# this-Demir/3D-Ray-Tracer-Vulkan

Hardware: AMD Instinct MI355X
Metric: Mrays/s at 1920×1080×4-bounce, 50k-tri scene; 1/2/4/8 GPU + %HBM roofline (higher is better)
Workload: dtype f32

## Files before the change

### 3d-ray-tracer-vulkan_amd/csrc/rt_internal.h

```cpp
#pragma once
#include <cstdint>
#include <cstddef>
#include <hip/hip_runtime.h>

#include "../../include/rtamd.h"

namespace rtamd {

constexpr int kShadeStride = 2;

struct DevScene {
    int      n_nodes = 0;
    int      end     = 0;
    int      n_tris  = 0;
    int      root_leaf = 0;
    float    root_box[6] = {0, 0, 0, 0, 0, 0};
    float4*  nodes   = nullptr;
    float4*  leafs   = nullptr;
    float4*  pairs   = nullptr;
    float4*  walk    = nullptr;
    int*     slot_node = nullptr;
    int*     node_slot = nullptr;
    int      end2    = 0;
    int      padded  = 0;
// ... 5 lines not shown
    int      root_enter = 0;
    int      root_first_leaf = 0;
    int      oct_mask = 7;
    float4*  walk_ref = nullptr;
    int      end2_ref = 0;
    int      ref_padded = 0;
    float4*  norms   = nullptr;
    float4*  mats    = nullptr;
    const float4* spheres = nullptr;
    int      n_spheres = 0;
};

struct Counters {
    unsigned long long segments;
    unsigned long long node_visits;
    unsigned long long tri_tests;
    unsigned long long mat_reads;
};

struct CamF {
    float ox, oy, oz;
    float lx, ly, lz;
    float hx, hy, hz;
    float vx, vy, vz;
};

constexpr int kExtSkyToggle = 1;
constexpr int kExtEmissive = 2;
constexpr int kExtAccumulate = 4;
constexpr int kExtSpheres = 8;
constexpr int kExtNewSample = 16;

constexpr int kMaxBatch = 16;

struct TraceArgs {
    DevScene scene;
    CamF     cams[kMaxBatch];
    int      n_frames;
    int      tiles_y;
    int      width, height;
    int      max_bounces;
    int      x0, y0, tw, th;
    int      band_h, band_stride, band_off;
    const int* band_list;
    uchar4*  out_rgba;
    float*   out_rad;
    Counters* counters;
    int      wave_tile;
    unsigned long long* diag;
    int      coop_lanes;
    int      solo_lanes;
    int      ext;
    int      sky_enabled;
    int      frame_count;
    float*   accum;
    int      walk;
    int      block_waves;
    const int* tile_order;
    int      tiles_x;
    int      split_n;
    int      heavy_tiles;
    int      heavy_fused;
    const int* heavy_px;
    int      n_heavy_px;
    const unsigned long long* tile_mask;
    unsigned* diag_lane;
    hipStream_t aux_stream;
    hipEvent_t ev_fork, ev_join;
    int      coop_walk;
    int      coop_win = 64;
    int      list_stride;
    const int* row_off = nullptr;
    int      split_bounce = 0;
    float4*  q_slots = nullptr;
    unsigned* q_count = nullptr;
    unsigned* q_prefix = nullptr;
    int      q_waves = 0;
    int      q_grid = 0;
    void*    q_temp = nullptr;
    size_t   q_temp_bytes = 0;
    const float4* ray_in = nullptr;
    float4*  hit_out = nullptr;
    int      any_hit = 0;
};

struct HostScene {
    int n_nodes = 0, end = 0, n_tris = 0, max_depth = 0, root_leaf = 0;
    float root_box[6] = {0, 0, 0, 0, 0, 0};
    float4* nodes = nullptr;
    float4* leafs = nullptr;
    float4* pairs = nullptr;
    float4* norms = nullptr;
    float4* mats  = nullptr;
};
int build_host_scene(const void* vertices, size_t vertex_bytes,
                     const void* materials, size_t material_bytes,
                     const void* bvh_nodes, size_t bvh_bytes,
                     HostScene* out, const char** err);
void free_host_scene(HostScene* s);

constexpr unsigned kLearnHeavyMark = 0x3FFFFFFFu;

struct LearnParams {
    int      n;
    int      rec_off;
    int      learn_cost;
    int      order_split;
    int      heavy_pixel_factor;
    int      concurrent;
    int      resident;
    int      cap;
    int      xcd = 0;
    int      tiles_x = 0, tiles_y = 0, frames = 0;
// ... 73 lines not shown
```

### 3d-ray-tracer-vulkan_amd/csrc/rt_runtime.hip

```cpp
#include "rt_internal.h"
#include <rocprim/device/device_scan.hpp>

#include "accel_build.h"

#include <cmath>
#include <cstdarg>
#include <cstdio>
#include <cstdlib>
#include <algorithm>
#include <cstring>
#include <new>
#include <string>
#include <vector>

namespace rtamd {

static thread_local char g_err[1024] = "";

void set_error(const char* fmt, ...) {
    va_list ap;
    va_start(ap, fmt);
    vsnprintf(g_err, sizeof g_err, fmt, ap);
    va_end(ap);
}

#define RT_HIP_CHECK(expr)                                                        \
    do {                                                                          \
        hipError_t e_ = (expr);                                                   \
        if (e_ != hipSuccess) {                                                   \
            set_error("%s failed: %s (%s:%d)", #expr, hipGetErrorString(e_),      \
                      __FILE__, __LINE__);                                        \
            return RT_ERR_HIP;                                                    \
        }                                                                         \
    } while (0)
// ... 208 lines not shown
                   bool pending = false;
                   void* d_base = nullptr;
                   int* d_nhpix = nullptr;
                   rt_learn_params given = {};
                   bool xcd_applied = false;
                   uint64_t seq = 0; };
    void*        d_learn_scratch = nullptr;
    size_t       learn_scratch_cap = 0;
    int*         h_nhpix = nullptr;
    hipEvent_t   learn_ev = nullptr;
    bool         learn_busy = false;
    bool         learn_oom = false;
    bool         learning_device = false;
    int          learning_rec_off = 0;
    uint64_t     learn_seq = 0;
    hipStream_t  aux[4] = {nullptr, nullptr, nullptr, nullptr};
    hipEvent_t   aux_fork[4] = {nullptr, nullptr, nullptr, nullptr}, aux_join[4] = {nullptr, nullptr, nullptr, nullptr};
    unsigned     aux_next = 0;
    std::vector<Order> orders;
    std::vector<uint8_t> learning_key;
    struct LastCam { std::vector<uint8_t> geo; std::vector<uint8_t> cam; };
    std::vector<LastCam> last_cam;
    size_t       learning_n = 0;
    int          learning_tx = 0, learning_ty = 0, learning_frames = 0;
    int          last_heavy = 0;
    int          last_heavy_px = 0;
    int          last_solo = 0;
    struct Graph { std::vector<uint64_t> key; hipGraphExec_t exec; int kernels; };
    uint64_t     plain_kernels = 0;
    struct BandList { std::vector<int> bands; int* d; };
    std::vector<BandList> band_lists;
    std::vector<Graph> graphs;
    unsigned     graph_next = 0;
    struct Slots { hipStream_t s; char* base; int waves; size_t temp_bytes; };
    std::vector<Slots> slots;
    char*        d_query = nullptr;
    size_t       query_cap = 0;
    int          ref_root_leaf = 0;
    char*        d_denoise = nullptr;
    size_t       denoise_cap = 0;
    char*        d_temporal = nullptr;
    size_t       temporal_cap = 0;
    bool         temporal_valid = false;
    int          temporal_last = 0, temporal_w = 0, temporal_h = 0;
    rt_camera_ubo temporal_cam = {};
    bool         moments_valid = false;
};

static constexpr size_t kMaxOrders = 16;
static constexpr int    kResidentPerCu = 24;
static constexpr int    kMaxHeavy = 256;
static constexpr size_t kWin32Bytes = 32ull << 20;
static constexpr size_t kSplitSlotBytes = 256ull << 20;
static constexpr unsigned kMaxWalkSlots = (1u << 27) - 4;
static constexpr size_t kDiagWords = 8;

static void free_order(PerDevice::Order& o) {
    if (o.d_base) {
        (void)hipFree(o.d_base);
        return;
    }
    (void)hipFree(o.d_order);
    if (o.d_hpix) (void)hipFree(o.d_hpix);
    if (o.d_mask) (void)hipFree(o.d_mask);
}

static void poll_learning(PerDevice& p) {
    if (!p.learn_busy || hipEventQuery(p.learn_ev) != hipSuccess) return;
    for (auto& o : p.orders)
        if (o.pending) {
            o.n_hpix = std::max(0, *p.h_nhpix);
            o.pending = false;
        }
    p.learn_busy = false;
}

static void free_orders(PerDevice& p) {
    for (auto& o : p.orders) free_order(o);
    p.orders.clear();
}

static void free_graphs(PerDevice& p) {
    for (auto& g : p.graphs) (void)hipGraphExecDestroy(g.exec);
    p.graphs.clear();
}
static constexpr size_t kMaxGraphs = 64;
// ... 5 lines not shown
    int  wave_tile = -1;
    int  diag = 0;
    int  coop_lanes = -1;
    int  solo_lanes = -1;
    int  ext = 0;
    int  new_sample = 0;
    int  walk = 2;
    int  coop_walk = 0;
    int  coop_window = 0;
    int  block_waves = 1;
    int  heavy_first = 1;
    int  heavy_factor = 130;
    int  heavy_pixels = 1;
    int  heavy_pixel_factor = 50;
    int  reuse_order = 1;
    int  heavy_cap = 75;
    int  async_slots = 4;
    int  copy_streams = 1;
    int  in_async = 0;
    int  concurrent_launches = 1;
    int  learn_cost = 1;
    int  learn_alone = 0;
    int  accel_octants = 7;
    int  xcd_order = 0;
    int  learn_device = 1;
    int  leaf_align = 2;
    int  accel_half = 0;
    int  accel_wide = 0;
    int  denoise_kernel = 0;
    int  denoise_pass = -1;
    int  temporal_tile = 0;
    int  variance_stage = -1;
    int  split_bounce = 0;
    int  accel = 8;
    int  order_split = 0;
    int  order_frames = 0;
    int  graph = 1;
    int  heavy_stream = 2;
    int  heavy_tiles = -1;
    uint64_t scene_gen = 0;
    int  hw_queues = 4;
    bool has_scene = false;
    int  n_nodes = 0, n_tris = 0, max_depth = 0;
    uint64_t issued = 0;
};

static void free_scene(PerDevice& p) {
    if (p.scene.nodes) (void)hipFree(p.scene.nodes);
    if (p.scene.leafs) (void)hipFree(p.scene.leafs);
    if (p.scene.walk) (void)hipFree(p.scene.walk);
    if (p.scene.walk_ref) (void)hipFree(p.scene.walk_ref);
    if (p.scene.slot_node) (void)hipFree(p.scene.slot_node);
    if (p.scene.node_slot) (void)hipFree(p.scene.node_slot);
    if (p.scene.pairs) (void)hipFree(p.scene.pairs);
    if (p.scene.norms) (void)hipFree(p.scene.norms);
    p.scene = DevScene{};
}

static int concurrency(const rt_ctx* ctx) { return std::max(ctx->concurrent_launches, ctx->in_async); }

static int plan_order(const rt_ctx* ctx, PerDevice& p, TraceArgs& a, const rt_camera_ubo* cams,
                      const std::vector<int>* bands) {
    a.tile_order = nullptr;
    a.tiles_x = 0;
    a.split_n = 0;
    a.heavy_tiles = 0;
// ... 359 lines not shown
        const size_t split = ctx->heavy_first ? (size_t)(ctx->heavy_tiles < 0 ? kMaxHeavy : ctx->heavy_tiles) * 63 : 0;
        const size_t words = (waves + split) * 8;
        if (words > p.diag_cap) {
            if (p.d_diag) {
                RT_HIP_CHECK(hipDeviceSynchronize());
                (void)hipFree(p.d_diag);
            }
            p.d_diag = nullptr;
            p.diag_cap = 0;
            RT_HIP_CHECK(hipMalloc(&p.d_diag, words * sizeof(unsigned long long)));
            p.diag_cap = words;
        }
        p.diag_used = words;
        a.diag = p.d_diag;
    }
    return plan_order(ctx, p, a, cam, bands);
}

static std::vector<uint64_t> launch_key(const TraceArgs& a, hipStream_t s) {
    auto P = [](const void* q) { return (uint64_t)(uintptr_t)q; };
    auto F = [](float f) { uint32_t u; std::memcpy(&u, &f, 4); return (uint64_t)u; };
    const DevScene& sc = a.scene;
    std::vector<uint64_t> k = {P(s), P(sc.nodes), P(sc.leafs), P(sc.pairs), P(sc.walk), P(sc.slot_node), P(sc.node_slot), P(sc.norms), P(sc.mats), P(sc.spheres),
            (uint64_t)sc.n_spheres, (uint64_t)sc.n_nodes, (uint64_t)sc.end, (uint64_t)sc.end2, (uint64_t)sc.n_tris,
            (uint64_t)sc.root_leaf, F(sc.root_box[0]), F(sc.root_box[1]), F(sc.root_box[2]), F(sc.root_box[3]),
            F(sc.root_box[4]), F(sc.root_box[5]), (uint64_t)a.n_frames, P(a.band_list), (uint64_t)a.list_stride,
            (uint64_t)a.width, (uint64_t)a.height, (uint64_t)a.max_bounces, (uint64_t)a.x0, (uint64_t)a.y0,
            (uint64_t)a.tw, (uint64_t)a.th, (uint64_t)a.band_h, (uint64_t)a.band_stride, (uint64_t)a.band_off,
            P(a.out_rgba), P(a.out_rad), (uint64_t)a.wave_tile,
            (uint64_t)a.coop_lanes, (uint64_t)a.solo_lanes, (uint64_t)a.ext, (uint64_t)a.sky_enabled,
            (uint64_t)a.frame_count, P(a.accum), (uint64_t)a.walk, (uint64_t)a.block_waves, P(a.tile_order),
            (uint64_t)a.heavy_tiles, (uint64_t)(a.aux_stream != nullptr), (uint64_t)a.heavy_fused, P(a.heavy_px),
            (uint64_t)a.n_heavy_px, P(a.tile_mask), (uint64_t)a.coop_walk, (uint64_t)a.coop_win,
            (uint64_t)a.split_bounce, P(a.q_slots), (uint64_t)a.q_waves, (uint64_t)a.q_grid};
    for (int f = 0; f < a.n_frames; ++f) {
        const CamF& c = a.cams[f];
        for (float v : {c.ox, c.oy, c.oz, c.lx, c.ly, c.lz, c.hx, c.hy, c.hz, c.vx, c.vy, c.vz}) k.push_back(F(v));
    }
    return k;
}

static int attach_slots(const rt_ctx* ctx, PerDevice& p, TraceArgs& a, hipStream_t s) {
    a.q_slots = nullptr;
    a.split_bounce = 0;
    if (!p.scene.n_layouts || ctx->split_bounce <= 0 || ctx->split_bounce >= a.max_bounces || a.ext || a.diag ||
        a.counters)
        return RT_OK;
    const int tw_w = 8 << a.wave_tile, th_w = 8 >> a.wave_tile, bw = std::max(1, a.block_waves);
    const long long waves = (long long)((a.tw + bw * tw_w - 1) / (bw * tw_w)) * bw *
                            ((a.th + th_w - 1) / th_w) * (long long)a.n_frames;
    if (waves > (1 << 24) || (size_t)waves * 64 * 48 > kSplitSlotBytes) return RT_OK;
    PerDevice::Slots* q = nullptr;
    for (auto& x : p.slots)
        if (x.s == s) { q = &x; break; }
    if (!q || q->waves < waves) {
        if (q) {
            RT_HIP_CHECK(hipStreamSynchronize(s));
            (void)hipFree(q->base);
            q->base = nullptr;
            q->waves = 0;
        } else {
            p.slots.push_back(PerDevice::Slots{s, nullptr, 0, 0});
            q = &p.slots.back();
        }
        size_t tb = 0;
        RT_HIP_CHECK(rocprim::exclusive_scan(nullptr, tb, (const unsigned*)nullptr, (unsigned*)nullptr, 0u,
                                             (size_t)waves, rocprim::plus<unsigned>()));
        void* base = nullptr;
        const size_t bytes = (size_t)waves * 64 * 48 + 2 * ((size_t)waves * 4 + 256) + tb + 256;
        RT_HIP_CHECK(hipMalloc(&base, bytes));
        q->base = static_cast<char*>(base);
        q->waves = (int)waves;
        q->temp_bytes = tb;
    }
    a.split_bounce = ctx->split_bounce;
    a.q_slots = reinterpret_cast<float4*>(q->base);
    a.q_count = reinterpret_cast<unsigned*>(q->base + (size_t)q->waves * 64 * 48);
    a.q_prefix = reinterpret_cast<unsigned*>(reinterpret_cast<char*>(a.q_count) + (size_t)q->waves * 4 + 256);
    a.q_temp = reinterpret_cast<char*>(a.q_prefix) + (size_t)q->waves * 4 + 256;
    a.q_temp_bytes = q->temp_bytes;
    a.q_waves = q->waves;
    a.q_grid = std::max(1, p.n_cu * 32);
    return RT_OK;
}

static int launch(const rt_ctx* ctx, PerDevice& p, const TraceArgs& a_in, hipStream_t s) {
    TraceArgs a = a_in;
    if (int rq = attach_slots(ctx, p, a, s)) return rq;
    const bool plain = !a.counters && !a.diag;
    int nk = 1;
    if (!ctx->graph || s == nullptr || a.counters || a.diag || !a.aux_stream) {
        RT_HIP_CHECK(launch_trace(a, s, &nk));
        if (plain) p.plain_kernels += (uint64_t)nk;
        return RT_OK;
    }
    std::vector<uint64_t> key = launch_key(a, s);
    for (auto& g : p.graphs)
        if (g.key == key) {
            RT_HIP_CHECK(hipGraphLaunch(g.exec, s));
            p.plain_kernels += g.kernels;
            return RT_OK;
        }
    hipGraph_t graph = nullptr;
    RT_HIP_CHECK(hipStreamBeginCapture(s, hipStreamCaptureModeThreadLocal));
    const hipError_t le = launch_trace(a, s, &nk);
    const hipError_t ce = hipStreamEndCapture(s, &graph);
    if (le != hipSuccess || ce != hipSuccess) {
        if (graph) (void)hipGraphDestroy(graph);
        set_error("graph capture: %s", hipGetErrorString(le != hipSuccess ? le : ce));
        return RT_ERR_HIP;
    }
    hipGraphExec_t exec = nullptr;
    const hipError_t ie = hipGraphInstantiate(&exec, graph, nullptr, nullptr, 0);
    (void)hipGraphDestroy(graph);
    if (ie != hipSuccess) { set_error("graph instantiate: %s", hipGetErrorString(ie)); return RT_ERR_HIP; }
    if (p.graphs.size() >= kMaxGraphs) {
        const size_t k = p.graph_next++ % kMaxGraphs;
        (void)hipGraphExecDestroy(p.graphs[k].exec);
        p.graphs[k] = PerDevice::Graph{std::move(key), exec, nk};
    } else {
        p.graphs.push_back(PerDevice::Graph{std::move(key), exec, nk});
    }
    RT_HIP_CHECK(hipGraphLaunch(exec, s));
    p.plain_kernels += (uint64_t)nk;
    return RT_OK;
}
// ... 1665 lines not shown
    return {name, field, 0, -1, 3, {a, b, c}};
}
static const Option kOptions[] = {
    in_range("coop_lanes", &rt_ctx::coop_lanes, -1, 64),
    in_range("solo_lanes", &rt_ctx::solo_lanes, -1, 64),
    in_range("extensions", &rt_ctx::ext, 0, 15),
    one_of("new_sample", &rt_ctx::new_sample, 0, 1),
    one_of("walk", &rt_ctx::walk, 0, 2),
    one_of("coop_window", &rt_ctx::coop_window, 0, 32, 64),
    one_of("coop_walk", &rt_ctx::coop_walk, 0, 1),
    one_of("block_waves", &rt_ctx::block_waves, 1, 4),
    one_of("heavy_first", &rt_ctx::heavy_first, 0, 1),
    in_range("heavy_tiles", &rt_ctx::heavy_tiles, -1, 1 << 20),
    in_range("heavy_factor", &rt_ctx::heavy_factor, 10, 100000),
    one_of("heavy_pixels", &rt_ctx::heavy_pixels, 0, 1),
    in_range("heavy_pixel_factor", &rt_ctx::heavy_pixel_factor, 1, 100000),
    one_of("reuse_order", &rt_ctx::reuse_order, 0, 1),
    in_range("heavy_cap", &rt_ctx::heavy_cap, 1, 100),
    in_range("async_slots", &rt_ctx::async_slots, 1, kMaxSlots),
    one_of("copy_streams", &rt_ctx::copy_streams, 1, 2),
    in_range("concurrent_launches", &rt_ctx::concurrent_launches, 1, 64),
    one_of("learn_cost", &rt_ctx::learn_cost, 0, 1),
    one_of("order_frames", &rt_ctx::order_frames, 0, 1),
    in_range("order_split", &rt_ctx::order_split, 0, 100),
    one_of("learn_alone", &rt_ctx::learn_alone, 0, 1),
    in_range("xcd_order", &rt_ctx::xcd_order, 0, 4096),
    in_range("accel_octants", &rt_ctx::accel_octants, 0, 7),
    one_of("learn_device", &rt_ctx::learn_device, 0, 1),
    in_range("leaf_align", &rt_ctx::leaf_align, 0, 2),
    one_of("accel", &rt_ctx::accel, 0, 1, 8),
    one_of("accel_half", &rt_ctx::accel_half, 0, 1),
    one_of("accel_wide", &rt_ctx::accel_wide, 0, 1),
    in_range("split_bounce", &rt_ctx::split_bounce, 0, 64),
    in_range("heavy_stream", &rt_ctx::heavy_stream, 0, 2),
    one_of("graph", &rt_ctx::graph, 0, 1),
    one_of("diag", &rt_ctx::diag, 0, 1),
    in_range("wave_tile", &rt_ctx::wave_tile, -1, 3),
    in_range("denoise_kernel", &rt_ctx::denoise_kernel, 0, 2),
    in_range("denoise_pass", &rt_ctx::denoise_pass, -1, 5),
    in_range("temporal_tile", &rt_ctx::temporal_tile, 0, 2),
    in_range("variance_stage", &rt_ctx::variance_stage, -1, 0),
};

static const Option* find_option(const char* name) {
    for (const Option& o : kOptions)
        if (std::strcmp(name, o.name) == 0) return &o;
    return nullptr;
}

int rt_set_option(rt_ctx* ctx, const char* name, int64_t value) {
    if (!ctx || !name) { set_error("rt_set_option: null argument"); return RT_ERR_INVALID_ARG; }
    static const char* const archived[] = {"shade_min", "blocks_per_cu", "seg_limit", "heavy_budget", "prio_after"};
    for (const char* a : archived)
        if (std::strcmp(name, a) == 0) {
            set_error("rt_set_option: %s belonged to a schedule archived in round 3 (profiles/r03/archive)", name);
            return RT_ERR_INVALID_ARG;
        }
    if (std::strcmp(name, "kernel") == 0 && value == 0) return RT_OK;
    if (const Option* o = find_option(name)) {
        bool ok = value >= o->lo && value <= o->hi;
        for (int k = 0; k < o->n; ++k) ok = ok || value == o->set[k];
        if (ok) {
            ctx->*(o->field) = (int)value;
            return RT_OK;
        }
    }
    set_error("rt_set_option: unknown option or bad value: %s = %lld", name, (long long)value);
    return RT_ERR_INVALID_ARG;
}

int rt_get_option(rt_ctx* ctx, const char* name, int64_t* value) {
    if (!ctx || !name || !value) { set_error("rt_get_option: null argument"); return RT_ERR_INVALID_ARG; }
    if (const Option* o = find_option(name)) {
        *value = ctx->*(o->field);
        return RT_OK;
    }
    const auto is = [name](const char* s) { return std::strcmp(name, s) == 0; };
    PerDevice* p = ctx->dev.empty() ? nullptr : &ctx->dev[0];
    if (is("kernel")) *value = 0;
    else if (is("wave_tile_used")) *value = p ? wave_tile_of(ctx, *p) : 0;
    else if (is("coop_window_used")) *value = p ? coop_window_of(ctx, *p) : 0;
    else if (is("accel_half_used")) *value = p ? p->scene.half : 0;
    else if (is("accel_wide_used")) *value = p ? p->scene.wide : 0;
    else if (is("accel_used")) *value = p ? p->scene.n_layouts : 0;
    else if (is("walk_bytes")) *value = p ? (int64_t)walk_bytes(*p) : 0;
    else if (is("leaf_align_used")) *value = p ? p->scene.padded : 0;
    else if (is("heavy_pixels_used")) *value = p ? p->last_heavy_px : 0;
    else if (is("heavy_tiles_used")) *value = p ? p->last_heavy : 0;
    else if (is("solo_lanes_used")) *value = p ? p->last_solo : 0;
    else if (is("plain_kernels")) *value = p ? (int64_t)p->plain_kernels : 0;
    else if (is("hw_queues")) *value = ctx->hw_queues;
    else if (is("queues_short")) *value = ctx->async_slots + 2 > ctx->hw_queues ? 1 : 0;
    else { set_error("rt_get_option: unknown option %s", name); return RT_ERR_INVALID_ARG; }
    return RT_OK;
}

int rt_diag_copy(rt_ctx* ctx, void* dst, size_t cap_words, size_t* n_words) {
    if (!ctx || !n_words) { set_error("rt_diag_copy: null argument"); return RT_ERR_INVALID_ARG; }
    PerDevice& p = ctx->dev[0];
    *n_words = p.diag_used;
    if (dst && p.d_diag && p.diag_used) {
        RT_HIP_CHECK(hipSetDevice(p.device));
        RT_HIP_CHECK(hipDeviceSynchronize());
        RT_HIP_CHECK(hipMemcpy(dst, p.d_diag, std::min(cap_words, p.diag_used) * 8, hipMemcpyDeviceToHost));
    }
    return RT_OK;
}

int rt_learn_device(rt_ctx* ctx, const void* d_records, const void* d_lanes, int n_tiles, const rt_learn_params* params,
                    void* d_order, void* d_mask, void* d_hpix, void* d_count, void* stream) {
    if (!ctx || !d_records || !d_lanes || !params || !d_order || !d_mask || !d_count) {
        set_error("rt_learn_device: null argument");
        return RT_ERR_INVALID_ARG;
    }
    const rt_learn_params& g = *params;
    if (n_tiles < 1 || n_tiles > (1 << 24) || g.rec_off < 0 || g.rec_off > (1 << 24) || (g.learn_cost & ~1) ||
        g.order_split < 0 || g.order_split > 100 || g.heavy_pixel_factor < 1 || g.concurrent < 1 || g.resident < 1 ||
        g.cap < 0 || g.xcd < 0 || g.tiles_x < 0 || g.tiles_y < 0 || g.frames < 0 || (g.cap > 0 && !d_hpix)) {
        set_error("rt_learn_device: bad tile count or parameters");
        return RT_ERR_INVALID_ARG;
    }
    PerDevice& p = ctx->dev[0];
    RT_HIP_CHECK(hipSetDevice(p.device));
// ... 139 lines not shown
```

### 3d-ray-tracer-vulkan_amd/csrc/rt_trace.hip

```cpp
#include <algorithm>
#include <cstdio>
#include <cstdlib>
#include <cstring>

#include <rocprim/device/device_scan.hpp>

#include "rt_internal.h"

namespace rtamd {

namespace {

constexpr float kTMin = 0.001f;
constexpr float kTMax = 10000.0f;
constexpr int   kMaxRejectTriples = 1 << 16;

struct V3 { float x, y, z; };

__device__ __forceinline__ V3 vadd(V3 a, V3 b) { return {a.x + b.x, a.y + b.y, a.z + b.z}; }
__device__ __forceinline__ V3 vsub(V3 a, V3 b) { return {a.x - b.x, a.y - b.y, a.z - b.z}; }
__device__ __forceinline__ V3 vmul(V3 a, V3 b) { return {a.x * b.x, a.y * b.y, a.z * b.z}; }
__device__ __forceinline__ V3 vscale(V3 a, float s) { return {a.x * s, a.y * s, a.z * s}; }
__device__ __forceinline__ float vdot(V3 a, V3 b) { return (a.x * b.x + a.y * b.y) + a.z * b.z; }
__device__ __forceinline__ V3 vcross(V3 a, V3 b) {
    return {a.y * b.z - a.z * b.y, a.z * b.x - a.x * b.z, a.x * b.y - a.y * b.x};
}
__device__ __forceinline__ V3 vnormalize(V3 a) {
    const float l = sqrtf(vdot(a, a));
    return {a.x / l, a.y / l, a.z / l};
}

__device__ __forceinline__ uint32_t pcg(uint32_t v) {
    const uint32_t s = v * 747796405u + 2891336453u;
    const uint32_t w = ((s >> ((s >> 28u) + 4u)) ^ s) * 277803737u;
    return (w >> 22u) ^ w;
}
__device__ __forceinline__ float rnd(uint32_t& seed) {
    seed = pcg(seed);
// ... 729 lines not shown
            }
        }
        sl = nl;
        if (!(sb < se)) break;
        if (QRY && any_hit && ((__ballot(hit >= 0 && !incons) >> L) & 1ull) != 0ull) break;
    }
    if (me) {
        if (COUNT) {
            c_node += cn;
            c_tri += ct;
        }
        if (DIAG) d_iters += steps;
    }
}

constexpr int kWavesPerEu = 8;
constexpr int kWalkPrio = 2;
template <bool COUNT, bool DIAG = false, int FEAT = 0, int WALK = 2>
__global__ __launch_bounds__(256)
__attribute__((amdgpu_waves_per_eu((FEAT & kFeatFrontier) ? 1 : kWavesPerEu)))
void trace_simple(TraceArgs a) {
    constexpr bool ACC = (FEAT & kFeatAccel) != 0;
    constexpr bool HALF = ACC && (FEAT & kFeatHalf) != 0;
    constexpr bool WIDE = ACC && (FEAT & kFeatWide) != 0;
    constexpr bool PAD = !ACC && ((FEAT & kFeatPad) || (FEAT & (kFeatExt | kFeatFrontier)) || !(FEAT & kFeatCoopTail));
    constexpr bool Q1 = (FEAT & kFeatQ1) != 0, Q2 = (FEAT & kFeatQ2) != 0;
    constexpr bool QRY = (FEAT & kFeatQuery) != 0;
    constexpr bool SOLO = (FEAT & kFeatSolo) != 0;
    static_assert(!SOLO || (ACC && !HALF && !WIDE && WALK == 2 && !(FEAT & (kFeatCoopTail | kFeatExt))),
                  "kFeatSolo goes with the format-0 accel walk alone");
    const int lane = threadIdx.x & 63;
    const int wave = threadIdx.x >> 6;
    extern __shared__ uint4 fr[];
    unsigned q_k = Q2 ? blockIdx.x : 0u;
    const unsigned q_total = Q2 ? a.q_prefix[a.q_waves - 1] + a.q_count[a.q_waves - 1] : 0u;
    if (Q2 && q_k * 64u >= q_total) return;
    const int s = a.wave_tile;
    const int tw_w = 8 << s, th_w = 8 >> s;
    int bx = blockIdx.x, by = blockIdx.y, sub = -1;
    if (QRY) {
        by = bx / a.tiles_x;
        bx -= by * a.tiles_x;
    }
    unsigned long long skip_lanes = 0;
    const int k_wave = (blockIdx.y * gridDim.x + blockIdx.x) * a.block_waves + wave;
    int rec_id = k_wave, tile_id = k_wave, hq = -1;
    if (a.tile_order) {
        const int k = blockIdx.x;
        int t;
        if ((FEAT & kFeatFused) && k < a.n_heavy_px) {
            hq = a.heavy_px[k];
            t = hq >> 6;
            sub = hq & 63;
        } else if (k < 64 * a.split_n) {
            t = a.tile_order[k >> 6];
            sub = k & 63;
        } else {
            t = a.tile_order[k - 63 * a.split_n - ((FEAT & kFeatFused) ? a.n_heavy_px : 0)];
            if ((FEAT & kFeatFused) && a.tile_mask) skip_lanes = a.tile_mask[t];
            if (FEAT & kFeatFused) {
                rec_id = a.n_heavy_px + t;
                tile_id = t;
            } else if (DIAG && a.diag_lane && a.split_n == 0) {
                rec_id = t;
                tile_id = t;
            }
        }
        bx = t % a.tiles_x;
        by = t / a.tiles_x;
    }
    unsigned long long* drec = nullptr;
    if (DIAG) {
        drec = a.diag + kDiagWords * (size_t)rec_id;
        diag_stamp(drec, 0);
    }
    if ((FEAT & kFeatFused) && sub >= 0) {
        const int hf = by / a.tiles_y;
        const int hy = (by - hf * a.tiles_y) * th_w + (sub >> (3 + s));
        heavy_pixel<COUNT>(a, hf, bx * tw_w + (sub & (tw_w - 1)), hy, (a.row_off ? a.row_off[hf] : hf * a.th) + hy, fr);
        if (DIAG) {
            diag_stamp(drec, 1);
            if (lane == 0) {
                drec[4] = 0;
                drec[5] = 0;
                drec[6] = 0;
                drec[7] = 0;
                if (a.diag_lane && hq >= 0) a.diag_lane[hq] = kHeavyLaneMark;
            }
        }
        return;
    }
    const int tl = sub >= 0 ? sub : lane;
    const int col = bx * a.block_waves + wave;
    const int fr_i = by / a.tiles_y;
    by -= fr_i * a.tiles_y;
    int lx = col * tw_w + (tl & (tw_w - 1));
    const int ly = by * th_w + (tl >> (3 + s));
    int lyo = (a.row_off ? a.row_off[fr_i] : fr_i * a.th) + ly;
    const bool pixel = !Q2 && lx < a.tw && ly < a.th && (sub < 0 || lane == 0) && !((skip_lanes >> lane) & 1ull) &&
                       (a.list_stride == 0 || a.band_list[fr_i * a.list_stride + ly / a.band_h] >= 0);
    if (Q1 && lane == 0) a.q_count[k_wave] = 0u;
    const int coop_lanes = sub >= 0 ? 64 : a.coop_lanes;
    const float4* __restrict__ nodes = a.scene.nodes;
    const float4* __restrict__ leafs = a.scene.leafs;
    const float4* __restrict__ pairs = a.scene.pairs;
    const int end = a.scene.end;
    const int wend = WALK == 2 ? a.scene.end2 : end;
    unsigned long long c_seg = 0, c_node = 0, c_tri = 0, c_mat = 0;
    unsigned long long d_iters = 0, d_windows = 0, d_coop_t = 0;
    unsigned long long d_lane_windows = 0;

  do {
    uint32_t seed = 0;
    V3 o = {0.f, 0.f, 0.f}, d = {0.f, 0.f, 1.f};
    V3 att = {1.0f, 1.0f, 1.0f};
    bool alive = pixel;
    int b0 = 0;
    float tmax = kTMax;
    bool refq = false;
    if (Q2) {
        const unsigned i = q_k * 64u + (unsigned)lane;
        alive = i < q_total;
        b0 = a.split_bounce;
        if (alive) {
            int lo = 0, hi = a.q_waves;
            while (hi - lo > 1) {
                const int mid = (lo + hi) >> 1;
                if (a.q_prefix[mid] <= i) lo = mid;
                else hi = mid;
            }
            const float4* r = a.q_slots + 3 * ((size_t)lo * 64 + (i - a.q_prefix[lo]));
            const float4 r0 = r[0], r1 = r[1], r2 = r[2];
            o = {r0.x, r0.y, r0.z};
            d = {r0.w, r1.x, r1.y};
            att = {r1.z, r1.w, r2.x};
            seed = __float_as_uint(r2.y);
            const int pq = __float_as_int(r2.z);
            lyo = pq / a.tw;
            lx = pq - lyo * a.tw;
        }
    }
    if (QRY && a.ray_in) {
        if (pixel) {
            const float4 r0 = a.ray_in[2 * (size_t)lx], r1 = a.ray_in[2 * (size_t)lx + 1];
            o = {r0.x, r0.y, r0.z};
            d = {r1.x, r1.y, r1.z};
            if (r0.w < kTMax) tmax = r0.w;
            if (!finite3(o) || !finite3(d) || (d.x == 0.0f && d.y == 0.0f && d.z == 0.0f)) {
                store_hit(a.hit_out + 2 * (size_t)lx, 0.0f, -2, V3{0.f, 0.f, 0.f}, V3{0.f, 0.f, 0.f});
                alive = false;
            }
            refq = ACC && fabsf(vdot(d, d) - 1.0f) > kRelaxAbs;
        }
    } else if (pixel) {
        const int x = a.x0 + lx, y = frame_row(a, fr_i, ly);
        if ((FEAT & kFeatExt) && (a.ext & (kExtAccumulate | kExtNewSample))) {
            seed = (uint32_t)(y * a.width + x) + (uint32_t)a.frame_count * (uint32_t)(a.width * a.height);
            primary_ray_seeded(a, fr_i, x, y, seed, o, d);
        } else {
            primary_ray(a, fr_i, x, y, seed, o, d);
        }
    }

    for (int b = b0; b < (QRY ? 1 : a.max_bounces); ++b) {
        if (__ballot(alive) == 0) break;
        if (Q1 && b == a.split_bounce) {
            const uint64_t m = __ballot(alive);
            if (alive) {
                float4* r = a.q_slots + 3 * ((size_t)k_wave * 64 + (size_t)lanes_below(m));
                r[0] = make_float4(o.x, o.y, o.z, d.x);
                r[1] = make_float4(d.y, d.z, att.x, att.y);
                r[2] = make_float4(att.z, __uint_as_float(seed), __int_as_float(lyo * a.tw + lx), 0.0f);
            }
            if (lane == 0) a.q_count[k_wave] = (unsigned)__popcll(m);
            alive = false;
            break;
        }
        float closest = QRY ? tmax : kTMax;
        int hit = -1;
        const V3 inv = {1.0f / d.x, 1.0f / d.y, 1.0f / d.z};
        int n = 0;
        int lend = wend;
        bool incons = false;
        int oct = 0;
        if (ACC && a.scene.n_layouts == 8) {
            oct = (int)((__float_as_uint(d.x) >> 31) | ((__float_as_uint(d.y) >> 31) << 1) |
                        ((__float_as_uint(d.z) >> 31) << 2)) & a.scene.oct_mask;
            n = oct * a.scene.layout_slots;
            lend = n + a.scene.layout_slots;
        }
        bool nleaf = a.scene.root_leaf != 0;
        const bool own = alive && !(QRY && refq);
        bool walking = own && end > 0;
        if (ACC && !HALF && !WIDE && a.scene.root_enter) {
            n += 1;
            nleaf = ((a.scene.root_first_leaf >> oct) & 1) != 0;
            if (COUNT && own) c_node += 2;
        }
        uint32_t wcur = a.scene.root_leaf ? kWLeaf : 0u;
        int wsp = 0;
        bool wovf = false;
        if (COUNT && alive) {
            ++c_seg;
            if (end > 0 && own) ++c_node;
        }
        {
            float4 A, B, Q0, Q1;
            const float4* __restrict__ wr = a.scene.walk;
            const __amdgpu_buffer_rsrc_t wrs = __builtin_amdgcn_make_buffer_rsrc(
// ... 227 lines not shown
            if ((FEAT & kFeatExt) ? hit != -1 : hit >= 0) {
                if (COUNT) ++c_mat;
                const V3 hp = vadd(o, vscale(d, closest));
                V3 nrm;
                float4 M;
                if ((FEAT & kFeatExt) && hit < -1) {
                    nrm = sphere_normal(a.scene.spheres[2 * (-2 - hit)], hp, d);
                    M = a.scene.spheres[2 * (-2 - hit) + 1];
                } else {
                    nrm = hit_normal(a.scene.norms, hit, d);
                    M = a.scene.mats[kShadeStride * hit];
                }
                V3 nd;
                if ((FEAT & kFeatExt) && (a.ext & kExtEmissive) && M.w == 3.0f) {
                    fin = vmul(att, V3{M.x, M.y, M.z});
                    alive = false;
                } else if (!scatter(M, d, nrm, seed, nd)) {
                    alive = false;
                } else {
                    att = vmul(att, V3{M.x, M.y, M.z});
                    o = hp;
                    d = nd;
                    if (b == a.max_bounces - 1) alive = false;
                }
            } else {
                if (!((FEAT & kFeatExt) && (a.ext & kExtSkyToggle) && a.sky_enabled == 0))
                    fin = vmul(att, sky_color(d));
                alive = false;
            }
            if (!alive) finish_pixel<FEAT>(a, lx, lyo, fin);
        }
    }
    if (!QRY && alive) finish_pixel<FEAT>(a, lx, lyo, V3{0.0f, 0.0f, 0.0f});
    q_k += gridDim.x;
  } while (Q2 && q_k * 64u < q_total);
    if (COUNT) flush_counters(a.counters, c_seg, c_node, c_tri, c_mat);
    if (DIAG) {
        diag_stamp(drec, 1);
        if (a.diag_lane && !((skip_lanes >> lane) & 1ull))
            a.diag_lane[(size_t)tile_id * 64 + lane] = (unsigned)(d_iters + 2 * d_lane_windows);
        unsigned long long d_sum = d_iters;
#pragma unroll
        for (int off = 32; off > 0; off >>= 1) {
            d_sum += __shfl_xor(d_sum, off);
            const unsigned long long o2 = __shfl_xor(d_iters, off);
            d_iters = o2 > d_iters ? o2 : d_iters;
        }
        if (lane == 0) {
            drec[4] = d_iters;
            drec[5] = d_windows;
            drec[6] = d_coop_t;
            drec[7] = d_sum;
        }
    }
}

}

#define RT_FUSED(G)                                                                                           \
    if (a.diag) hipLaunchKernelGGL((trace_simple<false, true, FF, 2>), G, block, shm, stream, ao);             \
    else if (a.counters) hipLaunchKernelGGL((trace_simple<true, false, FF, 2>), G, block, shm, stream, ao);     \
    else hipLaunchKernelGGL((trace_simple<false, false, FF, 2>), G, block, shm, stream, ao);
#define RT_FUSED_BIG(G)                                                                                       \
    switch (big) {                                                                                            \
        case kFeatWin32: { constexpr int FF = kFeatCoopTail | kFeatFused | kFeatWin32; RT_FUSED(G) } break;   \
        case kFeatPad: { constexpr int FF = kFeatCoopTail | kFeatFused | kFeatPad; RT_FUSED(G) } break;       \
        case kFeatWin32 | kFeatPad: {                                                                         \
            constexpr int FF = kFeatCoopTail | kFeatFused | kFeatWin32 | kFeatPad;                            \
// ... 47 lines not shown
                if (e != hipSuccess) return e;
            }
            TraceArgs ah = ao;
            ah.split_n = H;
            ah.coop_walk = 1;
            const dim3 gh(64 * H);
            const size_t shm = kFCap * sizeof(uint4);
            constexpr int FH = kFeatCoopTail | kFeatFrontier;
            if (a.diag) hipLaunchKernelGGL((trace_simple<false, true, FH, 2>), gh, block, shm, hs, ah);
            else if (a.counters) hipLaunchKernelGGL((trace_simple<true, false, FH, 2>), gh, block, shm, hs, ah);
            else hipLaunchKernelGGL((trace_simple<false, false, FH, 2>), gh, block, shm, hs, ah);
            e = hipGetLastError();
            if (e == hipSuccess && a.aux_stream) e = hipEventRecord(a.ev_join, a.aux_stream);
            if (e != hipSuccess) return e;
            if (kernels) *kernels = 2;
            ao.tile_order = a.tile_order + H;
            if (a.diag) ao.diag = a.diag + (size_t)kDiagWords * gh.x;
            grid = dim3(n_tiles - H);
            join = a.aux_stream != nullptr;
        } else {
            grid = dim3(n_tiles);
        }
    }
    const size_t shm_f = (size_t)bw * kFCap * sizeof(uint4);
    const size_t shm_w = (size_t)bw * kWideStackK * 64 * 6;
#define RT_SHM(F) (((F) & kFeatFrontier) ? shm_f : ((F) & kFeatWide) ? shm_w : 0)
#define RT_SIMPLE(F, W)                                                                                         \
    if (a.diag) hipLaunchKernelGGL((trace_simple<false, true, F, W>), grid, block, RT_SHM(F), stream, ao);           \
    else if (a.counters) hipLaunchKernelGGL((trace_simple<true, false, F, W>), grid, block, RT_SHM(F), stream, ao); \
    else hipLaunchKernelGGL((trace_simple<false, false, F, W>), grid, block, RT_SHM(F), stream, ao);
    if (a.scene.n_layouts > 0) {
        if (a.q_slots && a.split_bounce > 0 && a.split_bounce < a.max_bounces && feat == 0 && !a.scene.half &&
            !a.scene.wide &&
            !a.diag && !a.counters && (int)(grid.x * grid.y) * bw <= a.q_waves) {
            ao.q_waves = (int)(grid.x * grid.y) * bw;
            if (a.solo_lanes > 0)
                hipLaunchKernelGGL((trace_simple<false, false, kFeatAccel | kFeatQ1 | kFeatSolo, 2>), grid, block, 0,
                                   stream, ao);
            else
                hipLaunchKernelGGL((trace_simple<false, false, kFeatAccel | kFeatQ1, 2>), grid, block, 0, stream, ao);
            size_t tb = a.q_temp_bytes;
            const hipError_t se = rocprim::exclusive_scan(a.q_temp, tb, a.q_count, a.q_prefix, 0u,
                                                          (size_t)ao.q_waves, rocprim::plus<unsigned>(), stream);
            if (se != hipSuccess) return se;
            TraceArgs a2 = ao;
            a2.tile_order = nullptr;
            a2.split_n = 0;
            a2.block_waves = 1;
            if (a.solo_lanes > 0)
                hipLaunchKernelGGL((trace_simple<false, false, kFeatAccel | kFeatQ2 | kFeatSolo, 2>), dim3(a.q_grid),
                                   dim3(64), 0, stream, a2);
            else
                hipLaunchKernelGGL((trace_simple<false, false, kFeatAccel | kFeatQ2, 2>), dim3(a.q_grid), dim3(64), 0,
                                   stream, a2);
            if (kernels) *kernels = 2;
            return hipGetLastError();
        }
        if (a.scene.wide) {
            if (feat & kFeatCoopTail) {
                set_error("accel_wide launch with coop_lanes %d", a.coop_lanes);
                return hipErrorInvalidValue;
            }
            if (feat & kFeatExt) RT_SIMPLE(kFeatExt | kFeatAccel | kFeatWide, 2)
            else RT_SIMPLE(kFeatAccel | kFeatWide, 2)
            return hipGetLastError();
        }
        if (a.scene.half) {
            if (feat & kFeatCoopTail) {
                set_error("accel_half launch with coop_lanes %d", a.coop_lanes);
                return hipErrorInvalidValue;
            }
            if (feat & kFeatExt) RT_SIMPLE(kFeatExt | kFeatAccel | kFeatHalf, 2)
            else RT_SIMPLE(kFeatAccel | kFeatHalf, 2)
            return hipGetLastError();
        }
        switch (feat & ~kFeatFrontier) {
            case kFeatCoopTail:
                if (a.coop_win == 32) RT_SIMPLE(kFeatCoopTail | kFeatAccel | kFeatWin32, 2)
                else RT_SIMPLE(kFeatCoopTail | kFeatAccel, 2)
                break;
            case 0:
                if (a.solo_lanes > 0) RT_SIMPLE(kFeatAccel | kFeatSolo, 2)
                else RT_SIMPLE(kFeatAccel, 2)
                break;
            default: RT_SIMPLE(kFeatCoopTail | kFeatExt | kFeatAccel, 2) break;
        }
// ... 65 lines not shown
```

Measured before the change: 32550.

## Replace scan-based ray compaction with atomic bounded queues and auto-enable split

Wavefront ray compaction at the split bounce now appends surviving rays into a fixed set of bounded queues with atomic counters, replacing the per-wave count array, rocPRIM exclusive scan and binary-search lookup. The second pass launches one 64-lane block per queue pack, reads each ray directly, and resets the queue headers with a ticket counter, so no scan kernel or persistent loop is needed. Splitting at bounce 2 is also switched on by default for large frames with at least three bounces. Waves that find their queue full keep tracing in the first pass and bump an overflow counter. The risks are atomic contention, uneven fill across queues, and the new default changing which path runs.

```diff
diff --git a/3d-ray-tracer-vulkan_amd/csrc/rt_internal.h b/3d-ray-tracer-vulkan_amd/csrc/rt_internal.h
--- a/3d-ray-tracer-vulkan_amd/csrc/rt_internal.h
+++ b/3d-ray-tracer-vulkan_amd/csrc/rt_internal.h
@@ -61,6 +61,12 @@
 constexpr int kExtNewSample = 16;
 
 constexpr int kMaxBatch = 16;
+
+constexpr int kQHdrWords = 32;
+constexpr int kQCount = 0;
+constexpr int kQLimit = 1;
+constexpr int kQTicket = 2;
+constexpr int kMaxSplitQueues = 1024;
 
 struct TraceArgs {
     DevScene scene;
@@ -102,12 +108,13 @@
     const int* row_off = nullptr;
     int      split_bounce = 0;
     float4*  q_slots = nullptr;
-    unsigned* q_count = nullptr;
-    unsigned* q_prefix = nullptr;
-    int      q_waves = 0;
-    int      q_grid = 0;
-    void*    q_temp = nullptr;
-    size_t   q_temp_bytes = 0;
+    unsigned* q_hdr = nullptr;
+    unsigned* q_overflow = nullptr;
+    int      q_queues = 0;
+    int      q_cap = 0;
+    unsigned long long q_pixels = 0;
+    int      q_packs = 0;
+    int      q_spare = 0;
     const float4* ray_in = nullptr;
     float4*  hit_out = nullptr;
     int      any_hit = 0;
diff --git a/3d-ray-tracer-vulkan_amd/csrc/rt_runtime.hip b/3d-ray-tracer-vulkan_amd/csrc/rt_runtime.hip
--- a/3d-ray-tracer-vulkan_amd/csrc/rt_runtime.hip
+++ b/3d-ray-tracer-vulkan_amd/csrc/rt_runtime.hip
@@ -1,5 +1,4 @@
 #include "rt_internal.h"
-#include <rocprim/device/device_scan.hpp>
 
 #include "accel_build.h"
 
@@ -274,8 +273,9 @@
     std::vector<BandList> band_lists;
     std::vector<Graph> graphs;
     unsigned     graph_next = 0;
-    struct Slots { hipStream_t s; char* base; int waves; size_t temp_bytes; };
+    struct Slots { hipStream_t s; char* base; size_t bytes; };
     std::vector<Slots> slots;
+    int          last_split = 0;
     char*        d_query = nullptr;
     size_t       query_cap = 0;
     int          ref_root_leaf = 0;
@@ -294,6 +294,7 @@
 static constexpr int    kMaxHeavy = 256;
 static constexpr size_t kWin32Bytes = 32ull << 20;
 static constexpr size_t kSplitSlotBytes = 256ull << 20;
+static constexpr int kSplitPixelsDefault = 6000000;
 static constexpr unsigned kMaxWalkSlots = (1u << 27) - 4;
 static constexpr size_t kDiagWords = 8;
 
@@ -365,6 +366,9 @@
     int  temporal_tile = 0;
     int  variance_stage = -1;
     int  split_bounce = 0;
+    int  split_pixels = kSplitPixelsDefault;
+    int  split_queues = 256;
+    int  split_capacity = 64;
     int  accel = 8;
     int  order_split = 0;
     int  order_frames = 0;
@@ -790,7 +794,7 @@
             (uint64_t)a.frame_count, P(a.accum), (uint64_t)a.walk, (uint64_t)a.block_waves, P(a.tile_order),
             (uint64_t)a.heavy_tiles, (uint64_t)(a.aux_stream != nullptr), (uint64_t)a.heavy_fused, P(a.heavy_px),
             (uint64_t)a.n_heavy_px, P(a.tile_mask), (uint64_t)a.coop_walk, (uint64_t)a.coop_win,
-            (uint64_t)a.split_bounce, P(a.q_slots), (uint64_t)a.q_waves, (uint64_t)a.q_grid};
+            (uint64_t)a.split_bounce, P(a.q_slots), (uint64_t)a.q_queues, (uint64_t)a.q_cap};
     for (int f = 0; f < a.n_frames; ++f) {
         const CamF& c = a.cams[f];
         for (float v : {c.ox, c.oy, c.oz, c.lx, c.ly, c.lz, c.hx, c.hy, c.hz, c.vx, c.vy, c.vz}) k.push_back(F(v));
@@ -801,44 +805,50 @@
 static int attach_slots(const rt_ctx* ctx, PerDevice& p, TraceArgs& a, hipStream_t s) {
     a.q_slots = nullptr;
     a.split_bounce = 0;
-    if (!p.scene.n_layouts || ctx->split_bounce <= 0 || ctx->split_bounce >= a.max_bounces || a.ext || a.diag ||
-        a.counters)
+    a.q_queues = a.q_cap = a.q_packs = 0;
+    if (!p.scene.n_layouts || p.scene.half || p.scene.wide || a.coop_lanes > 0 || a.ext || a.diag || a.counters)
         return RT_OK;
     const int tw_w = 8 << a.wave_tile, th_w = 8 >> a.wave_tile, bw = std::max(1, a.block_waves);
     const long long waves = (long long)((a.tw + bw * tw_w - 1) / (bw * tw_w)) * bw *
                             ((a.th + th_w - 1) / th_w) * (long long)a.n_frames;
-    if (waves > (1 << 24) || (size_t)waves * 64 * 48 > kSplitSlotBytes) return RT_OK;
+    if (waves > (1 << 24)) return RT_OK;
+    const long long pixels = (long long)a.tw * a.th * a.n_frames;
+    int split = ctx->split_bounce;
+    if (split == 0 && ctx->split_pixels > 0 && a.max_bounces >= 3 && pixels >= ctx->split_pixels) split = 2;
+    if (split <= 0 || split >= a.max_bounces) return RT_OK;
+    const long long nq = std::max(1LL, std::min((long long)std::min(ctx->split_queues, kMaxSplitQueues), waves / 64));
+    const long long want = (waves * 64 * ctx->split_capacity + 1023) / 1024;
+    const long long cap = ctx->split_capacity > 0 ? ((want + nq - 1) / nq + 63) / 64 * 64 : 0;
+    const size_t bytes = (size_t)(nq * cap) * 48;
+    if (bytes > kSplitSlotBytes) return RT_OK;
+    const size_t hdr_bytes = (size_t)(kMaxSplitQueues + 1) * kQHdrWords * sizeof(unsigned);
     PerDevice::Slots* q = nullptr;
     for (auto& x : p.slots)
         if (x.s == s) { q = &x; break; }
-    if (!q || q->waves < waves) {
+    if (!q || q->bytes < bytes) {
         if (q) {
             RT_HIP_CHECK(hipStreamSynchronize(s));
             (void)hipFree(q->base);
             q->base = nullptr;
-            q->waves = 0;
+            q->bytes = 0;
         } else {
-            p.slots.push_back(PerDevice::Slots{s, nullptr, 0, 0});
+            p.slots.push_back(PerDevice::Slots{s, nullptr, 0});
             q = &p.slots.back();
         }
-        size_t tb = 0;
-        RT_HIP_CHECK(rocprim::exclusive_scan(nullptr, tb, (const unsigned*)nullptr, (unsigned*)nullptr, 0u,
-                                             (size_t)waves, rocprim::plus<unsigned>()));
         void* base = nullptr;
-        const size_t bytes = (size_t)waves * 64 * 48 + 2 * ((size_t)waves * 4 + 256) + tb + 256;
-        RT_HIP_CHECK(hipMalloc(&base, bytes));
+        RT_HIP_CHECK(hipMalloc(&base, hdr_bytes + bytes + 256));
+        RT_HIP_CHECK(hipMemsetAsync(base, 0, hdr_bytes, s));
         q->base = static_cast<char*>(base);
-        q->waves = (int)waves;
-        q->temp_bytes = tb;
-    }
-    a.split_bounce = ctx->split_bounce;
-    a.q_slots = reinterpret_cast<float4*>(q->base);
-    a.q_count = reinterpret_cast<unsigned*>(q->base + (size_t)q->waves * 64 * 48);
-    a.q_prefix = reinterpret_cast<unsigned*>(reinterpret_cast<char*>(a.q_count) + (size_t)q->waves * 4 + 256);
-    a.q_temp = reinterpret_cast<char*>(a.q_prefix) + (size_t)q->waves * 4 + 256;
-    a.q_temp_bytes = q->temp_bytes;
-    a.q_waves = q->waves;
-    a.q_grid = std::max(1, p.n_cu * 32);
+        q->bytes = bytes;
+    }
+    a.split_bounce = split;
+    a.q_hdr = reinterpret_cast<unsigned*>(q->base);
+    a.q_overflow = a.q_hdr + (size_t)kMaxSplitQueues * kQHdrWords;
+    a.q_slots = reinterpret_cast<float4*>(q->base + hdr_bytes);
+    a.q_queues = (int)nq;
+    a.q_cap = (int)cap;
+    a.q_packs = (int)std::max(1LL, cap / 64);
+    a.q_pixels = (unsigned long long)pixels;
     return RT_OK;
 }
 
@@ -847,9 +857,11 @@
     if (int rq = attach_slots(ctx, p, a, s)) return rq;
     const bool plain = !a.counters && !a.diag;
     int nk = 1;
+    p.last_split = 0;
     if (!ctx->graph || s == nullptr || a.counters || a.diag || !a.aux_stream) {
         RT_HIP_CHECK(launch_trace(a, s, &nk));
         if (plain) p.plain_kernels += (uint64_t)nk;
+        if (nk == 2 && a.q_slots) p.last_split = a.split_bounce;
         return RT_OK;
     }
     std::vector<uint64_t> key = launch_key(a, s);
@@ -2581,6 +2593,9 @@
     one_of("accel_half", &rt_ctx::accel_half, 0, 1),
     one_of("accel_wide", &rt_ctx::accel_wide, 0, 1),
     in_range("split_bounce", &rt_ctx::split_bounce, 0, 64),
+    in_range("split_pixels", &rt_ctx::split_pixels, 0, 1 << 30),
+    in_range("split_queues", &rt_ctx::split_queues, 1, kMaxSplitQueues),
+    in_range("split_capacity", &rt_ctx::split_capacity, 0, 1024),
     in_range("heavy_stream", &rt_ctx::heavy_stream, 0, 2),
     one_of("graph", &rt_ctx::graph, 0, 1),
     one_of("diag", &rt_ctx::diag, 0, 1),
@@ -2638,6 +2653,22 @@
     else if (is("heavy_tiles_used")) *value = p ? p->last_heavy : 0;
     else if (is("solo_lanes_used")) *value = p ? p->last_solo : 0;
     else if (is("plain_kernels")) *value = p ? (int64_t)p->plain_kernels : 0;
+    else if (is("split_bounce_used")) *value = p ? p->last_split : 0;
+    else if (is("split_overflow")) {
+        *value = 0;
+        for (PerDevice& d : ctx->dev) {
+            if (d.slots.empty()) continue;
+            RT_HIP_CHECK(hipSetDevice(d.device));
+            RT_HIP_CHECK(hipDeviceSynchronize());
+            for (auto& q : d.slots) {
+                unsigned* w = reinterpret_cast<unsigned*>(q.base) + (size_t)kMaxSplitQueues * kQHdrWords;
+                unsigned n = 0;
+                RT_HIP_CHECK(hipMemcpy(&n, w, sizeof n, hipMemcpyDeviceToHost));
+                RT_HIP_CHECK(hipMemset(w, 0, sizeof n));
+                *value += n;
+            }
+        }
+    }
     else if (is("hw_queues")) *value = ctx->hw_queues;
     else if (is("queues_short")) *value = ctx->async_slots + 2 > ctx->hw_queues ? 1 : 0;
     else { set_error("rt_get_option: unknown option %s", name); return RT_ERR_INVALID_ARG; }
diff --git a/3d-ray-tracer-vulkan_amd/csrc/rt_trace.hip b/3d-ray-tracer-vulkan_amd/csrc/rt_trace.hip
--- a/3d-ray-tracer-vulkan_amd/csrc/rt_trace.hip
+++ b/3d-ray-tracer-vulkan_amd/csrc/rt_trace.hip
@@ -2,8 +2,6 @@
 #include <cstdio>
 #include <cstdlib>
 #include <cstring>
-
-#include <rocprim/device/device_scan.hpp>
 
 #include "rt_internal.h"
 
@@ -799,9 +797,27 @@
     const int lane = threadIdx.x & 63;
     const int wave = threadIdx.x >> 6;
     extern __shared__ uint4 fr[];
-    unsigned q_k = Q2 ? blockIdx.x : 0u;
-    const unsigned q_total = Q2 ? a.q_prefix[a.q_waves - 1] + a.q_count[a.q_waves - 1] : 0u;
-    if (Q2 && q_k * 64u >= q_total) return;
+    unsigned q_first = 0u, q_valid = 0u;
+    if (Q2) {
+        const unsigned q = blockIdx.x % (unsigned)a.q_queues;
+        unsigned* const h = a.q_hdr + kQHdrWords * (size_t)q;
+        const unsigned cnt = __hip_atomic_load(h + kQCount, __ATOMIC_RELAXED, __HIP_MEMORY_SCOPE_AGENT);
+        const unsigned lim = ~__hip_atomic_load(h + kQLimit, __ATOMIC_RELAXED, __HIP_MEMORY_SCOPE_AGENT);
+        asm volatile("s_waitcnt vmcnt(0)" ::: "memory");
+        if (lane == 0) {
+            const unsigned t = __hip_atomic_fetch_add(h + kQTicket, 1u, __ATOMIC_RELAXED, __HIP_MEMORY_SCOPE_AGENT);
+            if (t + 1u == (unsigned)a.q_packs) {
+                __hip_atomic_store(h + kQCount, 0u, __ATOMIC_RELAXED, __HIP_MEMORY_SCOPE_AGENT);
+                __hip_atomic_store(h + kQLimit, 0u, __ATOMIC_RELAXED, __HIP_MEMORY_SCOPE_AGENT);
+                __hip_atomic_store(h + kQTicket, 0u, __ATOMIC_RELAXED, __HIP_MEMORY_SCOPE_AGENT);
+            }
+        }
+        q_valid = min(min(cnt, lim), (unsigned)a.q_cap);
+        q_first = (blockIdx.x / (unsigned)a.q_queues) * 64u;
+        if (q_first >= q_valid) return;
+        q_first += q * (unsigned)a.q_cap;
+        q_valid += q * (unsigned)a.q_cap;
+    }
     const int s = a.wave_tile;
     const int tw_w = 8 << s, th_w = 8 >> s;
     int bx = blockIdx.x, by = blockIdx.y, sub = -1;
@@ -866,7 +882,6 @@
     int lyo = (a.row_off ? a.row_off[fr_i] : fr_i * a.th) + ly;
     const bool pixel = !Q2 && lx < a.tw && ly < a.th && (sub < 0 || lane == 0) && !((skip_lanes >> lane) & 1ull) &&
                        (a.list_stride == 0 || a.band_list[fr_i * a.list_stride + ly / a.band_h] >= 0);
-    if (Q1 && lane == 0) a.q_count[k_wave] = 0u;
     const int coop_lanes = sub >= 0 ? 64 : a.coop_lanes;
     const float4* __restrict__ nodes = a.scene.nodes;
     const float4* __restrict__ leafs = a.scene.leafs;
@@ -877,7 +892,6 @@
     unsigned long long d_iters = 0, d_windows = 0, d_coop_t = 0;
     unsigned long long d_lane_windows = 0;
 
-  do {
     uint32_t seed = 0;
     V3 o = {0.f, 0.f, 0.f}, d = {0.f, 0.f, 1.f};
     V3 att = {1.0f, 1.0f, 1.0f};
@@ -886,25 +900,20 @@
     float tmax = kTMax;
     bool refq = false;
     if (Q2) {
-        const unsigned i = q_k * 64u + (unsigned)lane;
-        alive = i < q_total;
+        const unsigned i = q_first + (unsigned)lane;
+        alive = i < q_valid;
         b0 = a.split_bounce;
         if (alive) {
-            int lo = 0, hi = a.q_waves;
-            while (hi - lo > 1) {
-                const int mid = (lo + hi) >> 1;
-                if (a.q_prefix[mid] <= i) lo = mid;
-                else hi = mid;
-            }
-            const float4* r = a.q_slots + 3 * ((size_t)lo * 64 + (i - a.q_prefix[lo]));
+            const float4* r = a.q_slots + 3 * (size_t)i;
             const float4 r0 = r[0], r1 = r[1], r2 = r[2];
             o = {r0.x, r0.y, r0.z};
             d = {r0.w, r1.x, r1.y};
             att = {r1.z, r1.w, r2.x};
             seed = __float_as_uint(r2.y);
-            const int pq = __float_as_int(r2.z);
-            lyo = pq / a.tw;
-            lx = pq - lyo * a.tw;
+            const unsigned pq = __float_as_uint(r2.z);
+            alive = pq < a.q_pixels;
+            lyo = (int)(pq / (unsigned)a.tw);
+            lx = (int)(pq - (unsigned)lyo * (unsigned)a.tw);
         }
     }
     if (QRY && a.ray_in) {
@@ -933,15 +942,27 @@
         if (__ballot(alive) == 0) break;
         if (Q1 && b == a.split_bounce) {
             const uint64_t m = __ballot(alive);
-            if (alive) {
-                float4* r = a.q_slots + 3 * ((size_t)k_wave * 64 + (size_t)lanes_below(m));
-                r[0] = make_float4(o.x, o.y, o.z, d.x);
-                r[1] = make_float4(d.y, d.z, att.x, att.y);
-                r[2] = make_float4(att.z, __uint_as_float(seed), __int_as_float(lyo * a.tw + lx), 0.0f);
-            }
-            if (lane == 0) a.q_count[k_wave] = (unsigned)__popcll(m);
-            alive = false;
-            break;
+            const unsigned n = (unsigned)__popcll(m);
+            const unsigned q = (unsigned)k_wave % (unsigned)a.q_queues;
+            unsigned* const h = a.q_hdr + kQHdrWords * (size_t)q;
+            int base = 0;
+            if (lane == 0)
+                base = (int)__hip_atomic_fetch_add(h + kQCount, n, __ATOMIC_RELAXED, __HIP_MEMORY_SCOPE_AGENT);
+            base = lane_i(base, 0);
+            if ((unsigned long long)(unsigned)base + n <= (unsigned long long)(unsigned)a.q_cap) {
+                if (alive) {
+                    float4* r = a.q_slots + 3 * ((size_t)q * (size_t)a.q_cap + (unsigned)base + (size_t)lanes_below(m));
+                    r[0] = make_float4(o.x, o.y, o.z, d.x);
+                    r[1] = make_float4(d.y, d.z, att.x, att.y);
+                    r[2] = make_float4(att.z, __uint_as_float(seed), __int_as_float(lyo * a.tw + lx), 0.0f);
+                }
+                alive = false;
+                break;
+            }
+            if (lane == 0) {
+                __hip_atomic_fetch_max(h + kQLimit, ~(unsigned)base, __ATOMIC_RELAXED, __HIP_MEMORY_SCOPE_AGENT);
+                __hip_atomic_fetch_add(a.q_overflow, 1u, __ATOMIC_RELAXED, __HIP_MEMORY_SCOPE_AGENT);
+            }
         }
         float closest = QRY ? tmax : kTMax;
         int hit = -1;
@@ -1235,8 +1256,6 @@
         }
     }
     if (!QRY && alive) finish_pixel<FEAT>(a, lx, lyo, V3{0.0f, 0.0f, 0.0f});
-    q_k += gridDim.x;
-  } while (Q2 && q_k * 64u < q_total);
     if (COUNT) flush_counters(a.counters, c_seg, c_node, c_tri, c_mat);
     if (DIAG) {
         diag_stamp(drec, 1);
@@ -1350,26 +1369,22 @@
     if (a.scene.n_layouts > 0) {
         if (a.q_slots && a.split_bounce > 0 && a.split_bounce < a.max_bounces && feat == 0 && !a.scene.half &&
             !a.scene.wide &&
-            !a.diag && !a.counters && (int)(grid.x * grid.y) * bw <= a.q_waves) {
-            ao.q_waves = (int)(grid.x * grid.y) * bw;
+            !a.diag && !a.counters && a.q_queues > 0 && a.q_packs > 0) {
             if (a.solo_lanes > 0)
                 hipLaunchKernelGGL((trace_simple<false, false, kFeatAccel | kFeatQ1 | kFeatSolo, 2>), grid, block, 0,
                                    stream, ao);
             else
                 hipLaunchKernelGGL((trace_simple<false, false, kFeatAccel | kFeatQ1, 2>), grid, block, 0, stream, ao);
-            size_t tb = a.q_temp_bytes;
-            const hipError_t se = rocprim::exclusive_scan(a.q_temp, tb, a.q_count, a.q_prefix, 0u,
-                                                          (size_t)ao.q_waves, rocprim::plus<unsigned>(), stream);
-            if (se != hipSuccess) return se;
             TraceArgs a2 = ao;
             a2.tile_order = nullptr;
             a2.split_n = 0;
             a2.block_waves = 1;
+            const dim3 grid2((unsigned)a.q_queues * (unsigned)a.q_packs);
             if (a.solo_lanes > 0)
-                hipLaunchKernelGGL((trace_simple<false, false, kFeatAccel | kFeatQ2 | kFeatSolo, 2>), dim3(a.q_grid),
+                hipLaunchKernelGGL((trace_simple<false, false, kFeatAccel | kFeatQ2 | kFeatSolo, 2>), grid2,
                                    dim3(64), 0, stream, a2);
             else
-                hipLaunchKernelGGL((trace_simple<false, false, kFeatAccel | kFeatQ2, 2>), dim3(a.q_grid), dim3(64), 0,
+                hipLaunchKernelGGL((trace_simple<false, false, kFeatAccel | kFeatQ2, 2>), grid2, dim3(64), 0,
                                    stream, a2);
             if (kernels) *kernels = 2;
             return hipGetLastError();
```

After: 34860, median of 6. 1.07x the previous value.
